# ml-jku/LRAM

Hardware: AMD Instinct MI355X
Metric: env-steps/sec (action-inference) (higher is better)
Workload: dtype f32

## Files before the change

### lram_amd/csrc/common.h

```cpp
#pragma once
#include <hip/hip_runtime.h>
#include <stdint.h>

#include <stdexcept>
#include <string>

namespace lram {

inline bool first_use_on_device(uint64_t& mask) {
  int dev = 0;
  (void)hipGetDevice(&dev);
  const uint64_t bit = 1ull << (dev & 63);
  if (mask & bit) return false;
  mask |= bit;
  return true;
}

struct Error : std::runtime_error {
  using std::runtime_error::runtime_error;
};

#define LRAM_HIP_CHECK(expr)                                                                         \
  do {                                                                                               \
    hipError_t _e = (expr);                                                                          \
// ... 239 lines not shown
};
bool mlstm_front_supported(int inner, int NH, int K, int T);
void launch_mlstm_front(const MlstmFrontArgs& a, hipStream_t stream);
void launch_gate_coef(const float* wq, const float* wk, const float* wv, const float* wi, const float* wf, int inner, int NH,
                      float* gc, hipStream_t stream);
bool mlstm_chunk_supported(int inner, int NH, int K);
void launch_mlstm_chunk_pre(const MlstmPreArgs& a, hipStream_t stream);

struct MlstmCellArgs {
  float* C;
  const float* q;
  const float* k;
  const float* v;
  const float* scal;
  float* h;
  const uint8_t* reset;
  int B, T, NH, DH;
  int unroll = 8;
  int min_lds_bytes = 0;
  const float* amat = nullptr;
  const float* vec = nullptr;
  int chunk_exact_fp32 = 0;
};
void launch_mlstm_cell(const MlstmCellArgs& a, hipStream_t stream);
void launch_mlstm_chunk_cell(const MlstmCellArgs& a, hipStream_t stream);

constexpr int kLazyWindow = 48;
constexpr int kLazyWT = kLazyWindow + 4;
struct MlstmLazyArgs {
  float* C;
  float* wk;
  float* wv;
  const float* coef_in;
  float* coef_out;
  const float* g_in;
  float* g_out;
  const int32_t* count_in;
  int32_t* count_out;
  const float* q;
  const float* k;
  const float* v;
  const float* scal;
  float* h;
  const float *lean_xa = nullptr, *lean_u = nullptr, *lean_wq = nullptr, *lean_wk = nullptr, *lean_wv = nullptr;
  const float *gn_g = nullptr, *gn_b = nullptr, *gn_skip = nullptr;
  float gn_eps = 0.f;
  float* pw = nullptr;
  const uint8_t* reset;
  int B, T, NH, DH;
  int phase, period;
  int force;
  int compact = 0;
  int first = 0;
  int min_lds_bytes = 0;
};
void launch_mlstm_lazy_fold(const MlstmLazyArgs& a, hipStream_t stream);
void launch_mlstm_lazy_cell(const MlstmLazyArgs& a, hipStream_t stream);
bool mlstm_lazy_fused_scores(int DH);
void launch_mlstm_lazy_book(const MlstmLazyArgs& a, hipStream_t stream);
bool mlstm_lazy_supported(int DH, int T);
void launch_mlstm_lazy_clear(int32_t* count, float* g, const uint8_t* mask, int B, int NH, hipStream_t stream);
void launch_lazy_counts_as_float(const int32_t* count, float* out, int B, hipStream_t stream);

constexpr int kSlotChunk = 4096;
enum SlotSegKind : int32_t {
  kSlotSegState = 0,
  kSlotSegC = 1,
  kSlotSegSlstmY = 2,
  kSlotSegWindow = 3,
  kSlotSegCoef = 4,
  kSlotSegG = 5,
  kSlotSegCount = 6,
};
struct SlotSeg {
  float* base;
  int64_t stride;
  int64_t rec_off;
  int32_t numel;
  int32_t kind;
  int32_t parity;
  int32_t vec;
};
struct SlotChunk {
  int32_t seg, off;
};
struct SlotStateArgs {
  const SlotSeg* segs = nullptr;
  const SlotChunk* chunks = nullptr;
  int n_segs = 0, n_chunks = 0;
  const int32_t* src = nullptr;
  const int32_t* dst = nullptr;
  int n = 0;
  float* records = nullptr;
  int64_t rec_numel = 0;
  int lazy = 0, parity = 0;
  int rec_vec = 1;
};
void launch_slot_copy(const SlotStateArgs& a, hipStream_t stream);
void launch_slot_save(const SlotStateArgs& a, hipStream_t stream);
void launch_slot_load(const SlotStateArgs& a, hipStream_t stream);
void launch_slot_y_range(const SlotStateArgs& a, float limit, int* flag, hipStream_t stream);
struct SlotLazySaveArgs {
  const float *C = nullptr, *wk = nullptr, *wv = nullptr, *coef = nullptr, *g = nullptr;
  const int32_t* count = nullptr;
  const int32_t* slots = nullptr;
  int n = 0, NH = 0, DH = 0;
// ... 135 lines not shown
```

### lram_amd/csrc/engine.h

```cpp
#pragma once
#include <algorithm>
#include <array>
#include <cstdlib>
#include <cstring>
#include <map>
#include <memory>
#include <string>
#include <vector>

#include "../../include/lram_hip.h"
#include "common.h"

namespace lram::host {

struct DevBuf {
  float* p = nullptr;
  size_t n = 0;
  void alloc(size_t numel) {
    release();
    if (numel == 0) return;
    LRAM_HIP_CHECK(hipMalloc(reinterpret_cast<void**>(&p), numel * sizeof(float)));
    n = numel;
  }
  void zero(hipStream_t s = nullptr) {
// ... 70 lines not shown
  double gemm_counts[8] = {0, 0, 0, 0, 0, 0, 0, 0};
  std::vector<DevBuf> slstm_rt2;
  std::vector<DevBuf> slstm_rinv;
  int lazy_cap2_envs = 896;
  std::map<const float*, DevBuf> narrow;
  bool gemm_narrow_on = true;
  int gemm_narrow_min_rows = 256;
  bool upz_beside = true;
  bool slstm_gates_one = true;
  bool gemm_narrow_f16 = true;
  bool gn_amax_handover = true;
  bool gn_planes = true;
  bool slstm_seq_f32 = false;
  bool slstm_seq = true;
  std::vector<DevBuf> gate_coef;
  bool front_multi = true;
  int front_min_envs = 256;
  std::vector<DevBuf> dt_wt;
  DevBuf ASCALE;
  size_t ascale_rows = 0;
  DevBuf AMX_XN, AMX_XA, AMX_H;
  const float *w_state = nullptr, *b_state = nullptr, *w_rtg = nullptr, *b_rtg = nullptr, *w_rew = nullptr,
              *b_rew = nullptr, *eln_g = nullptr, *eln_b = nullptr, *w_head = nullptr, *b_head = nullptr,
              *post_g = nullptr, *post_b = nullptr;
  struct ImgConv {
    const float *w = nullptr, *b = nullptr;
    int cin = 0, cout = 0;
  };
  ImgConv img_conv[3][5];
  const float *img_lin_w = nullptr, *img_lin_b = nullptr;
  int img_channels = 0, img_flat = 0;
  DevBuf IMG_P, IMG_X0, IMG_X1, IMG_T;
  DevBuf IMG_EMB;
  static constexpr int fold_bubbles_images = 8;
  bool slot_table = false;
  std::vector<uint8_t> slot_flags, slot_act;
  std::vector<int32_t> slot_img_prefix;
  uint8_t* slot_dev = nullptr;
  int32_t* slot_img_list = nullptr;
  int slot_n_image = 0;
  bool slot_has_discrete = false;
  int lazy_mode = 2;
  bool lazy = false;
  bool lazy_ready = false;
  int lazy_period = 13;
  int gn_fuse = 2;
  bool mamba_dt_fuse = true;
  int slstm_fused_rows = 512;
  int gemm_skinny_rows = 384;
  static constexpr int slstm_gates_rows = 768;
  int gemm_skinny_min = 5;
  static constexpr int gemm_skinny_k = 1024;
  static constexpr int fold_bubbles = 2;
  int64_t lazy_step = 0;
  std::vector<int> lazy_bound;
  bool lazy_dirty = false;
  DevBuf LZ_COUNT;
  std::vector<SlotSeg> slot_segs;
  SlotSeg* slot_segs_dev = nullptr;
  SlotChunk* slot_chunks_dev = nullptr;
  int slot_n_chunks = 0, slot_n_rec_chunks = 0;
  int32_t* slot_idx_dev = nullptr;
  std::vector<int64_t> slot_c_off;
  bool slot_y_checked = false;
  void drop_slot_segments() {
    if (slot_segs_dev) (void)hipFree(slot_segs_dev);
    if (slot_chunks_dev) (void)hipFree(slot_chunks_dev);
    if (slot_idx_dev) (void)hipFree(slot_idx_dev);
    slot_segs_dev = nullptr, slot_chunks_dev = nullptr, slot_idx_dev = nullptr;
    slot_segs.clear(), slot_c_off.clear();
    slot_n_chunks = slot_n_rec_chunks = 0;
  }
  int B = 0;
  std::vector<BlockState> st;
  DevBuf X, XN, TOK, HID, U, Q, K, V, XA, H, G, SCAL, RY, LOGITS, RES, DTP;
  DevBuf XN2;
  DevBuf GATES, AMAT, VEC;
  DevBuf SEQ_EMB;
  DevBuf SCORE_LG;
  int score_rows = 4096;
  static constexpr int kScoreMinRows = 16;
  int last_head = -1;
  int tok_cap = 0;
  bool chunk_prefill = true;
  bool chunk_exact_fp32 = false;
  bool chunk_lanes = true;
  static constexpr int kMaxLanes = 3;
  static constexpr int n_lanes = 3;
  DevBuf twin[kMaxLanes - 1][21];
  std::vector<hipEvent_t> lane_ev[kMaxLanes];
  DevBuf SK;
  static constexpr size_t kSplitKSlotElems = 6u << 20;
  static constexpr int kSplitKSlots = 9;
  size_t ucols = 0, icols = 0;
  bool graph_mode = false;
  bool graph_valid = false;
  GraphKey graph_key{};
  hipGraph_t graph = nullptr;
  hipGraphExec_t graph_exec = nullptr;
  hipStream_t capture_stream = nullptr;
  int n_micro = 0;
  int compat_repeat = 1;
  DevBuf X0, U0;
  bool compat_share = true;
  bool compat_stale = false;
  bool sampling = false;
// ... 208 lines not shown
```

### lram_amd/csrc/engine.hip

```cpp
#include "engine.h"

namespace {

const float* need(lram_engine* e, const std::string& name, size_t numel) {
  auto it = e->weights.find(name);
  if (it == e->weights.end()) throw Error("lram: missing weight '" + name + "'");
  if (it->second.n != numel)
    throw Error("lram: weight '" + name + "' has " + std::to_string(it->second.n) + " elements, expected " +
                std::to_string(numel));
  return it->second.p;
}
const float* optional(lram_engine* e, const std::string& name, size_t numel) {
  auto it = e->weights.find(name);
  if (it == e->weights.end()) return nullptr;
  if (it->second.n != numel)
    throw Error("lram: weight '" + name + "' has " + std::to_string(it->second.n) + " elements, expected " +
                std::to_string(numel));
  return it->second.p;
}

void validate_config(const lram_config& c) {
  LRAM_REQUIRE(c.abi_version == LRAM_ABI_VERSION, "config.abi_version does not match the library");
  LRAM_REQUIRE(c.backbone == LRAM_BACKBONE_XLSTM || c.backbone == LRAM_BACKBONE_MAMBA, "unknown backbone");
  LRAM_REQUIRE(c.d_model > 0 && c.d_model % 4 == 0 && c.d_model <= 2048, "d_model must be a multiple of 4, <= 2048");
// ... 415 lines not shown
  const size_t B = e->B, NH = c.n_heads, DH = e->dh();
  for (int i = 0; i < c.n_blocks; ++i) {
    if (c.block_is_slstm[i]) continue;
    BlockState& s = e->st[i];
    s.wk.alloc(B * NH * kLazyWindow * DH);
    s.wv.alloc(B * NH * kLazyWindow * DH);
    s.coef.alloc(2 * B * NH * kLazyWindow);
    s.gsc.alloc(2 * B * NH);
    if (!mlstm_lazy_fused_scores((int)DH)) {
      s.pw.alloc(B * NH * 4 * kLazyWT);
      s.pw.zero();
    }
    s.coef.zero();
  }
  e->LZ_COUNT.alloc(2 * B);
  e->LZ_COUNT.zero();
  for (int i = 0; i < c.n_blocks; ++i) {
    if (c.block_is_slstm[i]) continue;
    BlockState& s = e->st[i];
    for (int p = 0; p < 2; ++p)
      launch_mlstm_lazy_clear(reinterpret_cast<int32_t*>(e->LZ_COUNT.p) + p * B, s.gsc.p + p * B * NH, nullptr, (int)B,
                              (int)NH, nullptr);
  }
  LRAM_HIP_CHECK(hipDeviceSynchronize());
  e->lazy_step = 0;
  e->lazy_ready = true;
  slot_segments_build(e);
}

bool lazy_choice(const lram_engine* e) {
  if (e->lazy_mode == 0 || !lazy_geometry_ok(e)) return false;
  if (e->lazy_mode == 1) return true;
  return mlstm_block_bytes(e) >= 128.0 * 1024 * 1024;
}

struct Knob {
  const char* name;
  void (*set)(lram_engine& e, const char* v);
};
const Knob kKnobs[] = {
    {"LRAM_STATE", [](lram_engine& e, const char* v) {
       const std::string m(v);
       e.lazy_mode = m == "lazy" ? 1 : (m == "eager" || m == "materialised" || m == "materialized") ? 0 : 2;
     }},
    {"LRAM_LAZY_PERIOD", [](lram_engine& e, const char* v) { e.lazy_period = std::max(1, std::min(14, std::atoi(v))); }},
    {"LRAM_LAZY_CAP2_ENVS", [](lram_engine& e, const char* v) { e.lazy_cap2_envs = std::max(0, std::atoi(v)); }},
    {"LRAM_GN_FUSE", [](lram_engine& e, const char* v) { e.gn_fuse = std::max(0, std::min(2, std::atoi(v))); }},
    {"LRAM_F16_MIN_ROWS", [](lram_engine& e, const char* v) { e.f16x2_min_rows = std::max(9, std::atoi(v)); }},
    {"LRAM_GEMM_PRESPLIT", [](lram_engine& e, const char* v) { e.gemm_presplit = std::atoi(v) != 0; }},
    {"LRAM_GEMM_NARROW", [](lram_engine& e, const char* v) { e.gemm_narrow_on = std::atoi(v) != 0, e.gemm_narrow_f16 = std::atoi(v) != 2; }},
    {"LRAM_UPZ_8P", [](lram_engine& e, const char* v) { e.upz_beside = std::atoi(v) != 0; }},
    {"LRAM_SLSTM_GATES_ONE", [](lram_engine& e, const char* v) { e.slstm_gates_one = std::atoi(v) != 0; }},
    {"LRAM_GN_AMAX", [](lram_engine& e, const char* v) { e.gn_amax_handover = std::atoi(v) != 0, e.gn_planes = std::atoi(v) >= 2; }},
    {"LRAM_GEMM_SKINNY_ROWS", [](lram_engine& e, const char* v) { e.gemm_skinny_rows = std::max(0, std::atoi(v)); }},
    {"LRAM_GEMM_SKINNY_MIN", [](lram_engine& e, const char* v) { e.gemm_skinny_min = std::max(1, std::atoi(v)); }},
    {"LRAM_SLSTM_FUSED_ROWS", [](lram_engine& e, const char* v) { e.slstm_fused_rows = std::max(0, std::atoi(v)); }},
    {"LRAM_SLSTM_SEQ", [](lram_engine& e, const char* v) { e.slstm_seq = std::atoi(v) != 0, e.slstm_seq_f32 = std::atoi(v) == 2; }},
    {"LRAM_FRONT_MULTI", [](lram_engine& e, const char* v) { e.front_multi = std::atoi(v) != 0; }},
    {"LRAM_FRONT_MIN_ENVS", [](lram_engine& e, const char* v) { e.front_min_envs = std::max(1, std::atoi(v)); }},
    {"LRAM_MAMBA_DT_FUSE", [](lram_engine& e, const char* v) { e.mamba_dt_fuse = std::atoi(v) != 0; }},
    {"LRAM_COMPAT_SHARE", [](lram_engine& e, const char* v) { e.compat_share = std::atoi(v) != 0; }},
    {"LRAM_PREFILL_CHUNK", [](lram_engine& e, const char* v) {
       e.chunk_prefill = std::atoi(v) != 0, e.chunk_exact_fp32 = std::atoi(v) == 2, e.chunk_lanes = std::atoi(v) != 3;
     }},
    {"LRAM_SCORE_ROWS", [](lram_engine& e, const char* v) { e.score_rows = std::max(lram_engine::kScoreMinRows, std::atoi(v)); }},
    {"LRAM_EVENT_SCOPE", [](lram_engine& e, const char* v) { e.event_device_scope = std::string(v) != "system"; }},
};

void state_alloc(lram_engine* e, int B) {
  LRAM_REQUIRE(e->finalized, "lram_finalize must be called before lram_state_alloc");
  LRAM_REQUIRE(B > 0 && B <= 65535, "batch must be in 1..65535");
  LRAM_HIP_CHECK(hipSetDevice(e->device));
  e->drop_graph();
  e->release_state();
  e->drop_slot_table();
  e->drop_sample_slots();
  const lram_config& c = e->cfg;
  const size_t D = c.d_model;
  e->st.resize(c.n_blocks);
  for (int i = 0; i < c.n_blocks; ++i) {
    BlockState& s = e->st[i];
    if (c.backbone == LRAM_BACKBONE_MAMBA) {
      s.s0.alloc((size_t)B * c.d_inner * c.d_state);
      s.conv.alloc((size_t)B * c.d_inner * c.d_conv);
    } else if (c.block_is_slstm[i]) {
      s.s0.alloc(4 * (size_t)B * D);
      s.conv.alloc((size_t)B * c.conv_k * D);
    } else {
      const size_t DH = e->dh();
      s.s0.alloc((size_t)B * c.n_heads * DH * DH);
      s.n.alloc((size_t)B * c.inner);
      s.m.alloc((size_t)B * c.n_heads);
      s.conv.alloc((size_t)B * c.conv_k * c.inner);
    }
    s.s0.zero();
    s.n.zero();
    s.m.zero();
    s.conv.zero();
  }
  e->B = B;
  alloc_workspace(e, kMaxTokens);
  e->lazy = lazy_choice(e);
  if (e->lazy) lazy_alloc(e);
  if (e->slot_segs_dev == nullptr) slot_segments_build(e);
  LRAM_HIP_CHECK(hipDeviceSynchronize());
}
// ... 251 lines not shown
```

### lram_amd/csrc/engine_xlstm.hip

```cpp
#include "engine.h"

namespace {

MlstmLazyArgs lazy_args(lram_engine* e, int i, int T, const uint8_t* reset, int b0, int nb) {
  const lram_config& c = e->cfg;
  const size_t NH = c.n_heads, DH = e->dh(), B = e->B;
  const int in = (int)(e->lazy_step & 1), out = 1 - in;
  BlockState& st = e->st[i];
  MlstmLazyArgs a{};
  a.C = st.s0.p + (size_t)b0 * NH * DH * DH;
  a.wk = st.wk.p + (size_t)b0 * NH * kLazyWindow * DH;
  a.wv = st.wv.p + (size_t)b0 * NH * kLazyWindow * DH;
  a.coef_in = st.coef.p + (in * B + b0) * NH * kLazyWindow;
  a.coef_out = st.coef.p + (out * B + b0) * NH * kLazyWindow;
  a.g_in = st.gsc.p + (in * B + b0) * NH;
  a.g_out = st.gsc.p + (out * B + b0) * NH;
  a.count_in = reinterpret_cast<const int32_t*>(e->LZ_COUNT.p) + in * B + b0;
  a.count_out = reinterpret_cast<int32_t*>(e->LZ_COUNT.p) + out * B + b0;
  a.pw = st.pw.p ? st.pw.p + (size_t)b0 * NH * T * kLazyWT : nullptr;
  a.reset = reset ? reset + b0 : nullptr;
  a.B = nb, a.T = T, a.NH = (int)NH, a.DH = (int)DH;
  a.phase = (int)((e->lazy_step + b0) % e->lazy_period), a.period = e->lazy_period, a.force = 0;
  return a;
}

}

namespace lram::host {

void lazy_materialize(lram_engine* e, hipStream_t s) {
  if (!e->lazy_ready || !e->lazy_dirty) return;
  const lram_config& c = e->cfg;
  const size_t B = e->B, NH = c.n_heads;
  for (int i = 0; i < c.n_blocks; ++i) {
    if (c.block_is_slstm[i]) continue;
    MlstmLazyArgs a = lazy_args(e, i, 1, nullptr, 0, e->B);
    a.force = 1;
    launch_mlstm_lazy_fold(a, s);
  }
  for (int i = 0; i < c.n_blocks; ++i) {
    if (c.block_is_slstm[i]) continue;
    for (int p = 0; p < 2; ++p)
      launch_mlstm_lazy_clear(reinterpret_cast<int32_t*>(e->LZ_COUNT.p) + p * B, e->st[i].gsc.p + p * B * NH, nullptr,
                              (int)B, (int)NH, s);
  }
  e->lazy_bound.assign(e->lazy_period, 0);
  e->lazy_dirty = false;
}

}

namespace {

bool lean_front(const lram_engine* e, int T) {
  return lazy_active(e, T) && mlstm_lazy_fused_scores(e->cfg.inner / e->cfg.n_heads);
}

bool split_up_now(const lram_engine* e) { return e->B >= 2048 && !e->graph_mode; }

bool gn_fused(const lram_engine* e, int T) {
  const int dh = e->cfg.inner / e->cfg.n_heads;
  return (e->gn_fuse == 1 || (e->gn_fuse == 2 && e->B >= 2048)) && lean_front(e, T) && e->use_bf16x3 && (dh == 256 || dh == 128) && T <= 4 &&
         e->cfg.inner % 8 == 0 && e->cfg.d_model % 8 == 0 && e->B >= 64;
}

void mlstm_front(lram_engine* e, const Pass& pass, int i, int T, const uint8_t* reset, const Slice& sl) {
  const lram_config& c = e->cfg;
  const int D = c.d_model, inner = c.inner, NH = c.n_heads, rows = sl.nb * T;
  const size_t r0 = (size_t)sl.b0 * T, b0 = sl.b0;
  const BlockWeights& w = e->bw[i];
  BlockState& st = e->st[i];
  float* amx = e->use_f16x2 ? e->AMX_XN.p + r0 : nullptr;
  GemmArgs up;
  up.a = e->XN.p + r0 * D, up.lda = D, up.w = w.proj_up, up.ldw = D, up.c = e->U.p + r0 * e->ucols, up.ldc = 2 * inner;
  up.m = rows, up.n = split_up_now(e) ? inner : 2 * inner, up.k = D;
// ... 201 lines not shown
    qa.gates = gates, qa.bias = w.rbias, qa.state = state, qa.yout = Y;
    if (e->slstm_rinv[i].p != nullptr)
      qa.rt2h = reinterpret_cast<const uint16_t*>(e->slstm_rt2[i].p), qa.rinv = e->slstm_rinv[i].p;
    else
      qa.rt2 = e->slstm_rt2[i].p;
    qa.B = sl.nb, qa.T = T, qa.H = Hs, qa.NH = NH, qa.state_B = e->B;
    launch_slstm_seq(qa, s);
  }
  for (int t = 0; !tok_fused && !seq && t < T; ++t) {
    GemmArgs ra;
    ra.a = state, ra.lda = Hs, ra.sA1 = SDH, ra.sA2 = 0;
    ra.w = w.rt, ra.ldw = SDH, ra.sW1 = 4 * (int64_t)SDH * SDH, ra.sW2 = (int64_t)SDH * SDH;
    ra.c = RY, ra.ldc = 4 * Hs, ra.sC1 = SDH, ra.sC2 = Hs;
    ra.m = sl.nb, ra.n = SDH, ra.k = SDH, ra.nb1 = NH, ra.nb2 = 4;
    gemm(e, ra, s);
    SlstmPointwiseArgs pw;
    pw.gates = gates, pw.ry = RY, pw.bias = w.rbias, pw.state = state, pw.yout = Y;
    pw.B = sl.nb, pw.T = T, pw.t = t, pw.H = Hs, pw.state_B = e->B;
    launch_slstm_pointwise(pw, s);
  }
  GroupNormArgs gn;
  gn.h = Y, gn.gamma = w.gn_g, gn.beta = w.gn_b, gn.out = X, gn.rows = rows, gn.NH = NH, gn.DH = SDH;
  gn.mode = 1, gn.eps = c.ln_eps, gn.skip = nullptr, gn.xa = nullptr, gn.u = nullptr;
  launch_group_norm(gn, s);
  float* amx = e->use_f16x2 ? e->AMX_XN.p + r0 : nullptr;
  GemmArgs up;
  up.a = XN, up.lda = D, up.w = w.ffn_up, up.ldw = D, up.c = Ubuf, up.ldc = 2 * F;
  up.m = rows, up.n = 2 * F, up.k = D;
  if (takes_skinny_with_norm(e, up)) {
    up.a = X, up.norm_g = w.ffn_norm_g, up.norm_b = w.ffn_norm_b, up.norm_eps = c.ln_eps, up.norm_rms = c.norm_is_rms;
    launch_gemm_skinny(up, s);
    count_gemm(e, 3, up);
  } else {
    launch_row_norm(X, D, XN, D, w.ffn_norm_g, w.ffn_norm_b, rows, D, c.ln_eps, c.norm_is_rms, s, nullptr, amx);
    up.a_amax = amx;
    gemm(e, up, s);
  }
  launch_gelu_gate(Ubuf, Gbuf, rows, F, s);
  GemmArgs dn;
  dn.a = Gbuf, dn.lda = F, dn.w = w.ffn_down, dn.ldw = F, dn.c = X, dn.ldc = D, dn.residual = X;
  dn.m = rows, dn.n = D, dn.k = F;
  gemm(e, dn, s);
}

}

namespace lram::host {

void run_xlstm_stack(lram_engine* e, const Pass& pass, int T, const uint8_t* reset, const std::vector<Slice>& sl, hipStream_t hbm) {
  const lram_config& c = e->cfg;
  const int D = c.d_model;
  const bool lazy = lazy_active(e, T);
  bool lazy_compact = false;
  if (lazy) {
    const int P = e->lazy_period;
    lazy_compact = true;
    if ((int)e->lazy_bound.size() != P) {
      e->lazy_bound.assign(P, kLazyWindow);
      lazy_compact = false;
    }
    const int c_due = (P - (int)(e->lazy_step % P)) % P;
    for (int cls = 0; cls < P; ++cls) {
      if (cls == c_due)
        e->lazy_bound[cls] = 0;
      else if (e->lazy_bound[cls] + T > kLazyWindow)
        lazy_compact = false;
      e->lazy_bound[cls] = std::min(e->lazy_bound[cls] + T, 4 * kLazyWindow);
    }
  }
  const bool bubbles = lazy && sl.size() > 1;
  const bool side_folds = lazy && sl.size() == 1 && e->n_micro == 0 && mlstm_block_bytes(e) >= 256.0 * 1024 * 1024;
  hipStream_t fold_stream = hbm;
  std::vector<hipEvent_t> fold_done(side_folds ? c.n_blocks : 0, nullptr);
  if (side_folds) {
    if (!e->hbm_stream) LRAM_HIP_CHECK(hipStreamCreateWithFlags(&e->hbm_stream, hipStreamNonBlocking));
    fold_stream = e->hbm_stream;
    stream_after(e, fold_stream, sl[0].s);
  }
  std::vector<char> folded(c.n_blocks, 0);
  auto launch_folds = [&](int i) {
    MlstmLazyArgs la = lazy_args(e, i, T, reset, 0, e->B);
    la.compact = lazy_compact ? 1 : 0;
    prof_record(e, fold_stream, true, true);
    launch_mlstm_lazy_fold(la, fold_stream);
    prof_record(e, fold_stream, false, true);
    folded[i] = 1;
  };
  auto next_mlstm = [&](int i) {
    for (int k = i + 1; k < c.n_blocks; ++k)
      if (!c.block_is_slstm[k]) return k;
    return -1;
  };
  if (bubbles) {
    int k = 0;
    const int ahead = pass.images != nullptr ? e->fold_bubbles_images : lram_engine::fold_bubbles;
    for (int i = next_mlstm(-1); i >= 0 && k < ahead; i = next_mlstm(i), ++k) launch_folds(i);
  }
  if (side_folds)
    for (int i = next_mlstm(-1); i >= 0; i = next_mlstm(i)) {
      launch_folds(i);
      fold_done[i] = ring_event(e);
      LRAM_HIP_CHECK(hipEventRecord(fold_done[i], fold_stream));
    }
  for (int i = 0; i < c.n_blocks; ++i) {
    if (i > 0 && pass.lane_rec) LRAM_HIP_CHECK(hipEventRecord((*pass.lane_rec)[i - 1], sl[0].s));
    if (pass.lane_wait) LRAM_HIP_CHECK(hipStreamWaitEvent(sl[0].s, (*pass.lane_wait)[i], 0));
    if (c.block_is_slstm[i]) {
      if (bubbles) {
        int left = 0, stretches = 0, must = 0;
        for (int k = next_mlstm(i); k >= 0; k = next_mlstm(k)) left += folded[k] ? 0 : 1;
        for (int k = i; k < c.n_blocks; ++k) stretches += c.block_is_slstm[k] ? 1 : 0;
        for (int k = i + 1; k < c.n_blocks && !c.block_is_slstm[k]; ++k) must += folded[k] ? 0 : 1;
        int take = left;
        if (stretches > 1) take = std::max((take + stretches - 1) / stretches, std::min(must, take));
        for (int k = next_mlstm(i); k >= 0 && take > 0; k = next_mlstm(k))
          if (!folded[k]) launch_folds(k), --take;
      }
      for (const Slice& x : sl) slstm_block(e, i, T, reset, x);
      continue;
    }
    if (lazy && !folded[i]) launch_folds(i);
    for (const Slice& x : sl) {
      mlstm_front(e, pass, i, T, reset, x);
      if (lazy) {
        MlstmLazyArgs la = lazy_args(e, i, T, reset, x.b0, x.nb);
        const size_t r0 = (size_t)x.b0 * T;
        la.q = e->Q.p + r0 * e->icols, la.k = e->K.p + r0 * e->icols, la.v = e->V.p + r0 * e->icols;
        la.scal = e->SCAL.p + r0 * c.n_heads * 4, la.h = e->H.p + r0 * e->icols;
        la.min_lds_bytes = (sl.size() >= 2 && x.nb <= e->lazy_cap2_envs && la.DH == 256) ? 54 * 1024 : 0;
        if (!mlstm_lazy_fused_scores(la.DH)) launch_mlstm_lazy_book(la, x.s);
        if (lean_front(e, T)) {
          const BlockWeights& w = e->bw[i];
          la.lean_xa = e->XA.p + r0 * e->icols, la.lean_u = e->U.p + r0 * e->ucols;
          la.lean_wq = w.wq, la.lean_wk = w.wk, la.lean_wv = w.wv;
          if (gn_fused(e, T)) la.gn_g = w.on_g, la.gn_b = w.on_b, la.gn_skip = w.skip, la.gn_eps = c.ln_eps;
// ... 31 lines not shown
```

### lram_amd/csrc/mlstm_lazy.hip

```cpp
#include <algorithm>
#include <cstdlib>

#include "common.h"
#include "device_math.h"

namespace lram {

typedef float f32x16 __attribute__((ext_vector_type(16)));
typedef float v4f __attribute__((ext_vector_type(4)));

namespace {

constexpr int W = kLazyWindow;

struct LazyView {
  int n_in;
  int n;
  bool fold;
  bool rs;
  bool zero_in;
  bool zero;
};

constexpr int kZeroBit = 1 << 16;
// ... 85 lines not shown
#pragma unroll
  for (int i = 0; i < (WF * (kFC / 4) + 255) / 256; ++i) {
    const int idx = tid + 256 * i;
    const int j = idx / (kFC / 4), c4 = (idx % (kFC / 4)) << 2;
    rv[i] = (idx < WF * (kFC / 4) && j < n) ? *reinterpret_cast<const float4*>(wvb + (int64_t)j * DH + c4) : f4_zero();
  }
  float4 rk[(WF * (kFR / 4) + 255) / 256];
  float rc[(WF * (kFR / 4) + 255) / 256];
#pragma unroll
  for (int i = 0; i < (WF * (kFR / 4) + 255) / 256; ++i) {
    const int idx = tid + 256 * i;
    const int j = idx / (kFR / 4), r4 = (idx % (kFR / 4)) << 2;
    const bool ok = idx < WF * (kFR / 4) && j < n;
    rk[i] = ok ? *reinterpret_cast<const float4*>(wkb + (int64_t)j * DH + r4) : f4_zero();
    rc[i] = ok ? cfb[j] : 0.f;
  }
#pragma unroll
  for (int i = 0; i < (WF * (kFC / 4) + 255) / 256; ++i) {
    const int idx = tid + 256 * i;
    if (idx < WF * (kFC / 4)) {
      const int j = idx / (kFC / 4), c4 = (idx % (kFC / 4)) << 2;
      *reinterpret_cast<float4*>(Vs + j * kFPV + c4) = rv[i];
    }
  }
#pragma unroll
  for (int i = 0; i < (WF * (kFR / 4) + 255) / 256; ++i) {
    const int idx = tid + 256 * i;
    if (idx < WF * (kFR / 4)) {
      const int j = idx / (kFR / 4), r4 = (idx % (kFR / 4)) << 2;
      const float cj = rc[i];
      *reinterpret_cast<float4*>(Ks + (r4 >> 5) * WF * kFPK + j * kFPK + (r4 & 31)) =
          make_float4(cj * rk[i].x, cj * rk[i].y, cj * rk[i].z, cj * rk[i].w);
    }
  }
  __syncthreads();
#pragma unroll
  for (int t = 0; t < kFR / 32; ++t) {
    f32x16 acc;
#pragma unroll
    for (int r = 0; r < 16; ++r) acc[r] = g * cold[t][r];
    const float* Kt = Ks + t * WF * kFPK;
    for (int j8 = 0; j8 < kt8; ++j8) {
#pragma unroll
      for (int i = 0; i < 4; ++i) {
        const int j = 8 * j8 + 4 * lh + i;
        acc = __builtin_amdgcn_mfma_f32_32x32x2f32(Kt[j * kFPK + li], Vs[j * kFPV + 32 * w + li], acc, 0, 0, 0);
      }
    }
#pragma unroll
    for (int r = 0; r < 16; ++r) cp0[(int64_t)(32 * t + (r & 3) + 8 * (r >> 2)) * DH] = acc[r];
  }
}

constexpr int WT = kLazyWT;


template <int T>
__global__ __launch_bounds__(256) void mlstm_lazy_score_kernel(MlstmLazyArgs a) {
  extern __shared__ float qk[];
  __shared__ float s_coef[W];
  const int h = blockIdx.x, b = blockIdx.y;
  const int tid = threadIdx.x, lane = tid & 63, wave = tid >> 6;
  const int NH = a.NH, DH = a.DH, inner = NH * DH;
  float* qs = qk;
  float* ks = qk + T * DH;
  LazyRaw raw = lazy_raw(a, b);
  const int64_t base = ((int64_t)b * NH + h) * W;
  const float coef_raw = tid < W ? a.coef_in[base + tid] : 0.f;
  float f[T], ig[T], F[T];
  float Fc = 1.f;
#pragma unroll
  for (int t = 0; t < T; ++t) {
    const float4 s = *reinterpret_cast<const float4*>(a.scal + (((int64_t)b * T + t) * NH + h) * 4);
    f[t] = s.x;
    ig[t] = s.y;
    Fc *= s.x;
    F[t] = Fc;
  }
  const float sqrt_dh = sqrtf((float)DH);
  {
    const int r4 = min(4 * tid, DH - 4);
    float4 qv[T], kv[T];
#pragma unroll
    for (int t = 0; t < T; ++t) {
      const int64_t off = ((int64_t)b * T + t) * inner + (int64_t)h * DH + r4;
      qv[t] = *reinterpret_cast<const float4*>(a.q + off);
      kv[t] = *reinterpret_cast<const float4*>(a.k + off);
    }
    if (4 * tid < DH) {
#pragma unroll
      for (int t = 0; t < T; ++t) {
        *reinterpret_cast<float4*>(qs + t * DH + r4) = qv[t];
        *reinterpret_cast<float4*>(ks + t * DH + r4) = make_float4(kv[t].x / sqrt_dh, kv[t].y / sqrt_dh, kv[t].z / sqrt_dh, kv[t].w / sqrt_dh);
      }
    }
    for (int r = 4 * (tid + 256); r < DH; r += 1024) {
#pragma unroll
      for (int t = 0; t < T; ++t) {
        const int64_t off = ((int64_t)b * T + t) * inner + (int64_t)h * DH + r;
        const float4 q4 = *reinterpret_cast<const float4*>(a.q + off), k4 = *reinterpret_cast<const float4*>(a.k + off);
        *reinterpret_cast<float4*>(qs + t * DH + r) = q4;
        *reinterpret_cast<float4*>(ks + t * DH + r) = make_float4(k4.x / sqrt_dh, k4.y / sqrt_dh, k4.z / sqrt_dh, k4.w / sqrt_dh);
      }
    }
  }
  __builtin_amdgcn_sched_barrier(0);
// ... 440 lines not shown
    if (tid < n) a.coef_out[base + tid] = s_coef[tid] * F[T - 1];
    if (tid < T) {
      float c = 1.f;
#pragma unroll
      for (int x = 0; x < T; ++x) {
        if (x == tid) c *= ig[x];
        if (x > tid) c *= f[x];
      }
      a.coef_out[base + n + tid] = c;
    }
    if (tid == 0) {
      a.g_out[(int64_t)b * NH + h] = g0 * F[T - 1];
      if (h == 0) a.count_out[b] = (n + T) | (lv.zero ? kZeroBit : 0);
    }
  }
}

__global__ __launch_bounds__(256) void mlstm_lazy_clear_kernel(int32_t* count, float* g, const uint8_t* mask, int B,
                                                               int NH) {
  const int gid = blockIdx.x * blockDim.x + threadIdx.x;
  if (gid >= B * NH) return;
  const int b = gid / NH;
  if (mask != nullptr && mask[b] == 0) return;
  g[gid] = 1.f;
  if (gid == b * NH) count[b] = 0;
}

template <int T, int LPR, int UNR, int KPL, int WP = W>
void launch_cell_tluk(const MlstmLazyArgs& a, hipStream_t s) {
  constexpr int CW = 4 * LPR, RP = 256 / LPR;
  dim3 grid(a.DH / CW, a.NH, a.B), block(256);
  size_t shmem = sizeof(float) * (2 * T * a.DH + RP * T * CW + T * kLazyWT + W + 8 * T);
  shmem = std::max(shmem, (size_t)a.min_lds_bytes);
  if (KPL == 4 && a.min_lds_bytes == 0) shmem = std::max(shmem, (size_t)41 * 1024);
  if (shmem > 48 * 1024) {
    static uint64_t raised = 0;
    if (first_use_on_device(raised)) {
      LRAM_HIP_CHECK(hipFuncSetAttribute(reinterpret_cast<const void*>(&mlstm_lazy_cell_kernel<T, LPR, UNR, KPL, WP>),
                                         hipFuncAttributeMaxDynamicSharedMemorySize, 160 * 1024));
    }
  }
  hipLaunchKernelGGL((mlstm_lazy_cell_kernel<T, LPR, UNR, KPL, WP>), grid, block, shmem, s, a);
}

template <int T>
void launch_cell_t(const MlstmLazyArgs& a, hipStream_t s) {
  if (a.DH == 256) return launch_cell_tluk<T, 64, 8, 4, 36>(a, s);
  if (a.DH == 128) return launch_cell_tluk<T, 32, 16, 0>(a, s);
  LRAM_REQUIRE(a.pw != nullptr, "lazy mLSTM: missing score buffer");
  if (a.DH % 256 == 0) return launch_cell_tluk<T, 64, 16, -1, 36>(a, s);
  launch_cell_tluk<T, 32, 16, -1, 36>(a, s);
}

}

bool mlstm_lazy_supported(int DH, int T) { return DH % 128 == 0 && T >= 1 && T <= 4; }

void launch_mlstm_lazy_fold(const MlstmLazyArgs& a_in, hipStream_t stream) {
  MlstmLazyArgs a = a_in;
  LRAM_REQUIRE(a.DH % kFC == 0 && a.DH % kFR == 0, "lazy mLSTM: head dim must be a multiple of 128");
  long envs = a.B;
  if (a.compact) {
    a.first = (a.period - a.phase % a.period) % a.period;
    if (a.first >= a.B) return;
    envs = (a.B - a.first + a.period - 1) / a.period;
  }
  const long nwg = envs * a.NH * (a.DH / kFC) * (a.DH / kFR);
  hipLaunchKernelGGL(mlstm_lazy_fold_kernel, dim3((unsigned)nwg), dim3(256), 0, stream, a);
  LRAM_HIP_CHECK(hipGetLastError());
}

bool mlstm_lazy_fused_scores(int DH) { return DH == 256 || DH == 128; }

void launch_mlstm_lazy_book(const MlstmLazyArgs& a, hipStream_t stream) {
  LRAM_REQUIRE(a.T >= 1 && a.T <= 4, "lazy mLSTM: 1..4 tokens per step");
  LRAM_REQUIRE(a.pw != nullptr, "lazy mLSTM: missing score buffer");
  dim3 grid(a.NH, a.B), block(256);
  const size_t shmem = sizeof(float) * 2 * a.T * a.DH;
  switch (a.T) {
    case 1: hipLaunchKernelGGL(mlstm_lazy_score_kernel<1>, grid, block, shmem, stream, a); break;
    case 2: hipLaunchKernelGGL(mlstm_lazy_score_kernel<2>, grid, block, shmem, stream, a); break;
    case 3: hipLaunchKernelGGL(mlstm_lazy_score_kernel<3>, grid, block, shmem, stream, a); break;
    default: hipLaunchKernelGGL(mlstm_lazy_score_kernel<4>, grid, block, shmem, stream, a); break;
  }
  LRAM_HIP_CHECK(hipGetLastError());
}

void launch_mlstm_lazy_cell(const MlstmLazyArgs& a, hipStream_t stream) {
  LRAM_REQUIRE(mlstm_lazy_supported(a.DH, a.T), "lazy mLSTM: unsupported geometry");
  switch (a.T) {
    case 1: launch_cell_t<1>(a, stream); break;
    case 2: launch_cell_t<2>(a, stream); break;
    case 3: launch_cell_t<3>(a, stream); break;
    default: launch_cell_t<4>(a, stream); break;
  }
  LRAM_HIP_CHECK(hipGetLastError());
}

void launch_mlstm_lazy_clear(int32_t* count, float* g, const uint8_t* mask, int B, int NH, hipStream_t stream) {
  hipLaunchKernelGGL(mlstm_lazy_clear_kernel, dim3((unsigned)((B * NH + 255) / 256)), dim3(256), 0, stream, count, g,
                     mask, B, NH);
  LRAM_HIP_CHECK(hipGetLastError());
}

namespace {
__global__ void lazy_counts_as_float_kernel(const int32_t* count, float* out, int B) {
  const int b = blockIdx.x * blockDim.x + threadIdx.x;
  if (b < B) out[b] = (float)(count[b] & 0xFFFF);
}
}

void launch_lazy_counts_as_float(const int32_t* count, float* out, int B, hipStream_t stream) {
  hipLaunchKernelGGL(lazy_counts_as_float_kernel, dim3((unsigned)((B + 255) / 256)), dim3(256), 0, stream, count, out, B);
  LRAM_HIP_CHECK(hipGetLastError());
}

}
```

Measured before the change: 460,800.

## Add wide lazy mLSTM fold kernel processing multiple row strips per workgroup

Adds a new fold kernel in which each workgroup handles S row strips of the C state, reusing the staged V window in LDS across strips. It prefetches the next strip's C and K while the current strip runs its MFMA work, and it writes output through an LDS transpose so stores are vectorised. When the due-class bound is small it uses a 40-row window variant, which cuts LDS use and raises the occupancy hint. This is on by default, and the old kernel stays reachable through an env knob. In exchange the grid is smaller, register pressure is higher, and the kernel relies on a host-tracked window bound.

```diff
diff --git a/lram_amd/csrc/common.h b/lram_amd/csrc/common.h
--- a/lram_amd/csrc/common.h
+++ b/lram_amd/csrc/common.h
@@ -315,6 +315,7 @@
   int force;
   int compact = 0;
   int first = 0;
+  int fold_form = 1, fold_strips = 2, fold_bound = 0;
   int min_lds_bytes = 0;
 };
 void launch_mlstm_lazy_fold(const MlstmLazyArgs& a, hipStream_t stream);
diff --git a/lram_amd/csrc/engine.h b/lram_amd/csrc/engine.h
--- a/lram_amd/csrc/engine.h
+++ b/lram_amd/csrc/engine.h
@@ -146,6 +146,9 @@
   int gemm_skinny_min = 5;
   static constexpr int gemm_skinny_k = 1024;
   static constexpr int fold_bubbles = 2;
+  bool fold_wide = true;
+  int fold_strips = 2;
+  bool fold_rows40 = true;
   int64_t lazy_step = 0;
   std::vector<int> lazy_bound;
   bool lazy_dirty = false;
diff --git a/lram_amd/csrc/engine.hip b/lram_amd/csrc/engine.hip
--- a/lram_amd/csrc/engine.hip
+++ b/lram_amd/csrc/engine.hip
@@ -491,6 +491,9 @@
     {"LRAM_UPZ_8P", [](lram_engine& e, const char* v) { e.upz_beside = std::atoi(v) != 0; }},
     {"LRAM_SLSTM_GATES_ONE", [](lram_engine& e, const char* v) { e.slstm_gates_one = std::atoi(v) != 0; }},
     {"LRAM_GN_AMAX", [](lram_engine& e, const char* v) { e.gn_amax_handover = std::atoi(v) != 0, e.gn_planes = std::atoi(v) >= 2; }},
+    {"LRAM_FOLD_KERNEL", [](lram_engine& e, const char* v) { e.fold_wide = std::atoi(v) != 0; }},
+    {"LRAM_FOLD_STRIPS", [](lram_engine& e, const char* v) { e.fold_strips = std::max(1, std::min(4, std::atoi(v))); }},
+    {"LRAM_FOLD_ROWS", [](lram_engine& e, const char* v) { e.fold_rows40 = std::atoi(v) < kLazyWindow; }},
     {"LRAM_GEMM_SKINNY_ROWS", [](lram_engine& e, const char* v) { e.gemm_skinny_rows = std::max(0, std::atoi(v)); }},
     {"LRAM_GEMM_SKINNY_MIN", [](lram_engine& e, const char* v) { e.gemm_skinny_min = std::max(1, std::atoi(v)); }},
     {"LRAM_SLSTM_FUSED_ROWS", [](lram_engine& e, const char* v) { e.slstm_fused_rows = std::max(0, std::atoi(v)); }},
diff --git a/lram_amd/csrc/engine_xlstm.hip b/lram_amd/csrc/engine_xlstm.hip
--- a/lram_amd/csrc/engine_xlstm.hip
+++ b/lram_amd/csrc/engine_xlstm.hip
@@ -21,6 +21,7 @@
   a.reset = reset ? reset + b0 : nullptr;
   a.B = nb, a.T = T, a.NH = (int)NH, a.DH = (int)DH;
   a.phase = (int)((e->lazy_step + b0) % e->lazy_period), a.period = e->lazy_period, a.force = 0;
+  a.fold_form = e->fold_wide ? 1 : 0, a.fold_strips = e->fold_strips;
   return a;
 }
 
@@ -328,6 +329,7 @@
   const int D = c.d_model;
   const bool lazy = lazy_active(e, T);
   bool lazy_compact = false;
+  int lazy_due_bound = 0;
   if (lazy) {
     const int P = e->lazy_period;
     lazy_compact = true;
@@ -336,6 +338,7 @@
       lazy_compact = false;
     }
     const int c_due = (P - (int)(e->lazy_step % P)) % P;
+    lazy_due_bound = (lazy_compact && e->fold_rows40) ? e->lazy_bound[c_due] : 0;
     for (int cls = 0; cls < P; ++cls) {
       if (cls == c_due)
         e->lazy_bound[cls] = 0;
@@ -357,6 +360,7 @@
   auto launch_folds = [&](int i) {
     MlstmLazyArgs la = lazy_args(e, i, T, reset, 0, e->B);
     la.compact = lazy_compact ? 1 : 0;
+    la.fold_bound = lazy_compact ? lazy_due_bound : 0;
     prof_record(e, fold_stream, true, true);
     launch_mlstm_lazy_fold(la, fold_stream);
     prof_record(e, fold_stream, false, true);
diff --git a/lram_amd/csrc/mlstm_lazy.hip b/lram_amd/csrc/mlstm_lazy.hip
--- a/lram_amd/csrc/mlstm_lazy.hip
+++ b/lram_amd/csrc/mlstm_lazy.hip
@@ -161,6 +161,146 @@
   }
 }
 
+constexpr int kFQ = 8;
+constexpr int kFPT = 32;
+template <int S, int WR, bool EARLY>
+__global__ __launch_bounds__(256, WR == 40 && S <= 2 ? 4 : 3) void mlstm_lazy_fold_wide_kernel(MlstmLazyArgs a) {
+  static_assert(WR % 8 == 0 && WR <= W, "window rows in LDS: a multiple of 8 up to the window capacity");
+  __shared__ __attribute__((aligned(16))) float Vs[WR * kFPV];
+  __shared__ __attribute__((aligned(16))) float Ks[(kFR / 32) * WR * kFPK];
+  __shared__ __attribute__((aligned(16))) float Ts[4 * kFQ * kFPT];
+  const int DH = a.DH, NH = a.NH;
+  const int nsl = DH / kFC;
+  int wid = blockIdx.x;
+  const int nwg = gridDim.x;
+  if ((nwg & 7) == 0) wid = (wid & 7) * (nwg >> 3) + (wid >> 3);
+  const int ngr = DH / (kFR * S);
+  const int grp = wid % ngr;
+  wid /= ngr;
+  const int slice = wid % nsl, bh = wid / nsl, h = bh % NH;
+  const int b = a.compact ? a.first + (bh / NH) * a.period : bh / NH;
+  if (b >= a.B) return;
+  const int tid = threadIdx.x, lane = tid & 63, w = tid >> 6, li = lane & 31, lh = lane >> 5;
+  const int lr = lane >> 3, lc = (lane & 7) << 2;
+  const int row0 = grp * S * kFR;
+  float* cp0 = a.C + (((int64_t)b * NH + h) * DH + row0 + lr) * DH + slice * kFC + 32 * w + lc;
+  float* Tw = Ts + w * kFQ * kFPT;
+  v4f cc[kFR / 32][4], cn[kFR / 32][4];
+  auto request_c = [&](v4f (&c)[kFR / 32][4], int s) {
+#pragma unroll
+    for (int t = 0; t < kFR / 32; ++t)
+#pragma unroll
+      for (int q = 0; q < 4; ++q) c[t][q] = *reinterpret_cast<const v4f*>(cp0 + (int64_t)(kFR * s + 32 * t + 8 * q) * DH);
+  };
+  LazyRaw raw = lazy_raw(a, b);
+  const float g_raw = a.g_in[(int64_t)b * NH + h];
+  if (EARLY) {
+    request_c(cc, 0);
+    __builtin_amdgcn_sched_barrier(0);
+    asm volatile("" : "+v"(raw.rb), "+v"(raw.word));
+  }
+  const LazyView lv = lazy_view_of(a, b, raw);
+  if (!lv.fold) return;
+  const int n = min(lv.n_in, WR);
+  const int kt8 = (n + 7) >> 3;
+  const bool zin = lv.zero_in;
+  const float g = zin ? 0.f : g_raw;
+  const float* wkb = a.wk + (((int64_t)b * NH + h) * W) * DH + row0;
+  const float* wvb = a.wv + (((int64_t)b * NH + h) * W) * DH + slice * kFC;
+  const float* cfb = a.coef_in + ((int64_t)b * NH + h) * W;
+  if (!EARLY && !zin) request_c(cc, 0);
+  constexpr int NV = (WR * (kFC / 4) + 255) / 256, NK = (WR * (kFR / 4) + 255) / 256;
+  float4 rv[NV];
+#pragma unroll
+  for (int i = 0; i < NV; ++i) {
+    const int idx = tid + 256 * i;
+    const int j = min(idx / (kFC / 4), n - 1), c4 = (idx % (kFC / 4)) << 2;
+    rv[i] = *reinterpret_cast<const float4*>(wvb + (int64_t)j * DH + c4);
+  }
+  float4 rk[NK];
+  float rc[NK];
+  auto request_k = [&](int s) {
+#pragma unroll
+    for (int i = 0; i < NK; ++i) {
+      const int idx = tid + 256 * i;
+      const int j = min(idx / (kFR / 4), n - 1), r4 = (idx % (kFR / 4)) << 2;
+      rk[i] = *reinterpret_cast<const float4*>(wkb + (int64_t)j * DH + kFR * s + r4);
+      rc[i] = cfb[j];
+    }
+  };
+  auto stage_k = [&]() {
+#pragma unroll
+    for (int i = 0; i < NK; ++i) {
+      const int idx = tid + 256 * i;
+      if (idx < WR * (kFR / 4)) {
+        const int j = idx / (kFR / 4), r4 = (idx % (kFR / 4)) << 2;
+        const float cj = rc[i];
+        *reinterpret_cast<float4*>(Ks + (r4 >> 5) * WR * kFPK + j * kFPK + (r4 & 31)) =
+            j < n ? make_float4(cj * rk[i].x, cj * rk[i].y, cj * rk[i].z, cj * rk[i].w) : f4_zero();
+      }
+    }
+  };
+  request_k(0);
+  __builtin_amdgcn_sched_barrier(0);
+#pragma unroll
+  for (int i = 0; i < NV; ++i) {
+    const int idx = tid + 256 * i;
+    if (idx < WR * (kFC / 4)) {
+      const int j = idx / (kFC / 4), c4 = (idx % (kFC / 4)) << 2;
+      *reinterpret_cast<float4*>(Vs + j * kFPV + c4) = j < n ? rv[i] : f4_zero();
+    }
+  }
+  stage_k();
+  __syncthreads();
+#pragma unroll
+  for (int s = 0; s < S; ++s) {
+    if (s + 1 < S) {
+      if (!zin) request_c(cn, s + 1);
+      request_k(s + 1);
+      __builtin_amdgcn_sched_barrier(0);
+    }
+#pragma unroll
+    for (int t = 0; t < kFR / 32; ++t) {
+      f32x16 acc;
+      if (zin) {
+#pragma unroll
+        for (int r = 0; r < 16; ++r) acc[r] = 0.f;
+      } else {
+#pragma unroll
+        for (int q = 0; q < 4; ++q) {
+          *reinterpret_cast<v4f*>(Tw + lr * kFPT + lc) = cc[t][q];
+#pragma unroll
+          for (int i = 0; i < 4; ++i) acc[4 * q + i] = g * Tw[(i + 4 * lh) * kFPT + li];
+        }
+      }
+      const float* Kt = Ks + t * WR * kFPK;
+      for (int j8 = 0; j8 < kt8; ++j8) {
+#pragma unroll
+        for (int i = 0; i < 4; ++i) {
+          const int j = 8 * j8 + 4 * lh + i;
+          acc = __builtin_amdgcn_mfma_f32_32x32x2f32(Kt[j * kFPK + li], Vs[j * kFPV + 32 * w + li], acc, 0, 0, 0);
+        }
+      }
+#pragma unroll
+      for (int q = 0; q < 4; ++q) {
+#pragma unroll
+        for (int i = 0; i < 4; ++i) Tw[(i + 4 * lh) * kFPT + li] = acc[4 * q + i];
+        const v4f o = *reinterpret_cast<const v4f*>(Tw + lr * kFPT + lc);
+        *reinterpret_cast<v4f*>(cp0 + (int64_t)(kFR * s + 32 * t + 8 * q) * DH) = o;
+      }
+    }
+    if (s + 1 < S) {
+      __syncthreads();
+      stage_k();
+#pragma unroll
+      for (int t = 0; t < kFR / 32; ++t)
+#pragma unroll
+        for (int q = 0; q < 4; ++q) cc[t][q] = cn[t][q];
+      __syncthreads();
+    }
+  }
+}
+
 constexpr int WT = kLazyWT;
 
 
@@ -707,6 +847,13 @@
   launch_cell_tluk<T, 32, 16, -1, 36>(a, s);
 }
 
+template <int WR, bool EARLY>
+void launch_fold_wide(int S, dim3 grid, const MlstmLazyArgs& a, hipStream_t s) {
+  if (S == 4) hipLaunchKernelGGL((mlstm_lazy_fold_wide_kernel<4, WR, EARLY>), grid, dim3(256), 0, s, a);
+  else if (S == 2) hipLaunchKernelGGL((mlstm_lazy_fold_wide_kernel<2, WR, EARLY>), grid, dim3(256), 0, s, a);
+  else hipLaunchKernelGGL((mlstm_lazy_fold_wide_kernel<1, WR, EARLY>), grid, dim3(256), 0, s, a);
+}
+
 }
 
 bool mlstm_lazy_supported(int DH, int T) { return DH % 128 == 0 && T >= 1 && T <= 4; }
@@ -720,8 +867,24 @@
     if (a.first >= a.B) return;
     envs = (a.B - a.first + a.period - 1) / a.period;
   }
-  const long nwg = envs * a.NH * (a.DH / kFC) * (a.DH / kFR);
-  hipLaunchKernelGGL(mlstm_lazy_fold_kernel, dim3((unsigned)nwg), dim3(256), 0, stream, a);
+  if (a.fold_form == 0) {
+    const long nwg = envs * a.NH * (a.DH / kFC) * (a.DH / kFR);
+    hipLaunchKernelGGL(mlstm_lazy_fold_kernel, dim3((unsigned)nwg), dim3(256), 0, stream, a);
+    LRAM_HIP_CHECK(hipGetLastError());
+    return;
+  }
+  const int strips = a.DH / kFR;
+  int S = a.fold_strips >= 4 ? 4 : a.fold_strips >= 2 ? 2 : 1;
+  while (strips % S != 0) S >>= 1;
+  const bool rows40 = a.compact != 0 && a.force == 0 && a.fold_bound > 0 && a.fold_bound <= 40;
+  const dim3 grid((unsigned)(envs * a.NH * (a.DH / kFC) * (strips / S)));
+  if (rows40) {
+    launch_fold_wide<40, true>(S, grid, a, stream);
+  } else if (a.compact != 0) {
+    launch_fold_wide<W, true>(S, grid, a, stream);
+  } else {
+    launch_fold_wide<W, false>(S, grid, a, stream);
+  }
   LRAM_HIP_CHECK(hipGetLastError());
 }
 
```

Result: no change. 464,800 (median of 6 runs) (+0.9%).
